# treangenlab/komb

Hardware: AMD Instinct MI355X
Metric: peeled edges/sec (k-truss) (higher is better)
Workload: dtype int32

## Files before the change

### komb_amd/csrc/ktruss.hip

```cpp
#include "peel_dev.h"
#include "truss_tail.h"
#include "local_dev.h"
#include "shard_dev.h"

#include <algorithm>
#include <cstdlib>
#include <cstring>

#include "truss_line.h"
#include "truss_tri.h"
#include "truss_wedge.h"
#include "truss_index.h"
#include "truss_gather.h"

namespace komb {

namespace {

struct TrussProblem {
    static constexpr bool kChain = false;
    static constexpr bool kSingleStep = false;
    uint32_t units;
    const uint2 *off2;
    const int2 *inc;
// ... 209 lines not shown
        }
        ctx->d_ceu = eu; ctx->d_cev = ev;
    }
    ctx->d_t_eu = ctx->d_ceu; ctx->d_t_ev = ctx->d_cev;
    return KOMB_OK;
}

int truss_support_canonical(komb_ctx *ctx)
{
    if (ctx->t_sup_ready) return KOMB_OK;
    if (!ctx->truss_done || !ctx->d_t_slice || !ctx->prep.valid || ctx->prep.ne != ctx->t_ne)
        KOMB_FAIL(ctx, KOMB_ERR_STATE, "komb_truss_fetch_support: no k-truss result to take the supports from");
    hipStream_t s = ctx->stream;
    const int64_t m = ctx->t_ne;
    KOMB_HIP(ctx, ctx->pool.get((void **)&ctx->d_t_sup, (size_t)m * sizeof(int32_t)));
#ifndef KOMB_TEST_SKIP_SLICE_ZERO
    if (ctx->t_k_lo) KOMB_HIP(ctx, hipMemsetAsync(ctx->d_t_sup, 0, (size_t)ctx->t_k_lo * sizeof(int32_t), s));
    if (ctx->t_k_hi < (uint32_t)m) KOMB_HIP(ctx, hipMemsetAsync(ctx->d_t_sup + ctx->t_k_hi, 0, ((size_t)m - ctx->t_k_hi) * sizeof(int32_t), s));
#endif
    k_scatter_len<<<grid_for(m), kBlock, 0, s>>>(ctx->d_t_slice, ctx->prep.e2k, m, ctx->t_k_lo, ctx->t_k_hi, ctx->d_t_sup);
    KOMB_HIP(ctx, hipStreamSynchronize(s));
    ctx->t_sup_ready = true;
    return KOMB_OK;
}

int truss_run(komb_ctx *ctx, const uint8_t *vmask_host, int rank, int world, komb_allreduce_fn fn, void *user)
{
    if (world < 1 || rank < 0 || rank >= world || (world > 1 && !fn))
        KOMB_FAIL(ctx, KOMB_ERR_ARG, "komb_truss_run_sharded: bad rank %d / world %d / callback", rank, world);
    if (ctx->nv < 0) KOMB_FAIL(ctx, KOMB_ERR_STATE, "komb_truss_run: no graph loaded");
    truss_free(ctx);
    hipStream_t s = ctx->stream;
    komb_stats &st = ctx->stats;
    st.triangles = 0; st.truss_levels = st.truss_subrounds = st.truss_launches = 0;
    st.max_trussness = 0; st.ms_support = st.ms_peel = st.ms_orient = st.ms_tri_count = st.ms_tri_fill = st.ms_gather = st.ms_allreduce = st.ms_compact = 0.0;
    st.truss_scans = 0; st.ms_prepare = 0.0; st.truss_prepared = 0; st.ms_prep_vertex = st.ms_prep_edges = st.ms_prep_rows = 0.0;
    auto empty_result = [&]() -> int {
        KOMB_HIP(ctx, ctx->pool.get((void **)&ctx->d_t_eu, 4)); KOMB_HIP(ctx, ctx->pool.get((void **)&ctx->d_t_ev, 4));
        KOMB_HIP(ctx, ctx->pool.get((void **)&ctx->d_t_truss, 4)); KOMB_HIP(ctx, ctx->pool.get((void **)&ctx->d_t_sup, 4));
        ctx->t_own_edges = true; ctx->t_ne = 0; ctx->truss_done = true; ctx->t_sup_ready = true;
        return KOMB_OK;
    };
    if (ctx->nv == 0 || ctx->ne == 0) return empty_result();
    Range r_all("komb_truss_run");
    DevBufs bufs(ctx);

    Range phase("truss: preparation");
    InducedCsr sub;
    TrussPrep sub_prep;
    struct SubGuard { komb_ctx *c; InducedCsr *g; TrussPrep *p; ~SubGuard() { prep_free(c, p); induced_free(c, g); } } sub_guard{ctx, &sub, &sub_prep};
    TrussPrep *tp = &ctx->prep;
    if (vmask_host) {
        ctx->timer.start(s);
        KOMB_TRY(induce_csr(ctx, vmask_host, &sub));
        st.ms_orient = ctx->timer.stop(s);
        if (sub.ns == 0) return empty_result();
        KOMB_TRY(prep_build(ctx, sub.rowptr, sub.col, sub.nv, sub.ns, &sub_prep));
        st.ms_prepare = sub_prep.ms; st.truss_prepared = 1;
        st.ms_prep_vertex = sub_prep.ms_part[0]; st.ms_prep_edges = sub_prep.ms_part[1]; st.ms_prep_rows = sub_prep.ms_part[2];
        tp = &sub_prep;
    } else if (!ctx->prep.valid) {
        KOMB_TRY(prep_ensure(ctx));
        st.ms_prepare = ctx->prep.ms; st.truss_prepared = 1;
        st.ms_prep_vertex = ctx->prep.ms_part[0]; st.ms_prep_edges = ctx->prep.ms_part[1]; st.ms_prep_rows = ctx->prep.ms_part[2];
    }
    const int64_t nv = tp->nv;
    const int64_t m = tp->ne;
    const uint32_t *d_orow = tp->orow;
    const int32_t *d_ocol = tp->ocol;
    const uint4 *d_line = tp->vline;
    const uint2 *d_wtasks = (const uint2 *)tp->wtasks;
    const int64_t n_wtasks = tp->n_wtasks;
    const int gw = grid_for(n_wtasks, kTriWaves);
    phase.next("truss: triangles + incidence index");

    const int ge = grid_for(m);
    const int tri_tv = (int)std::max<int64_t>(1, std::min<int64_t>(kTriV, nv / (256 * KOMB_TRI_EU * kTriWaves * 4)));
    const int64_t ntasks = (nv + tri_tv - 1) / tri_tv;
    const int gt = grid_for(ntasks, kTriWaves);
    uint32_t *d_own = nullptr, *d_other = nullptr, *d_cnt = nullptr, *d_off = nullptr;
    uint2 *d_off2 = nullptr;
    KOMB_HIP(ctx, bufs.alloc(&d_own, 2 * ((size_t)m + 1)));
    d_other = d_own + ((size_t)m + 1);
    KOMB_HIP(ctx, bufs.alloc(&d_cnt, (size_t)m + 1));
    KOMB_HIP(ctx, bufs.alloc(&d_off2, (size_t)m + 4));
    unsigned long long *d_mom = nullptr;
    KOMB_HIP(ctx, bufs.alloc(&d_mom, 12));
    KOMB_HIP(ctx, hipMemsetAsync(d_mom, 0, 12 * sizeof(unsigned long long), s));
    st.ms_allreduce = 0.0;

    const FinishMode fin = finish_mode(ctx, FIN_LOCAL);
    if (fin == FIN_LDS) KOMB_TRY(prep_sources(ctx, tp));
    const int32_t *d_osrc = tp->osrc;
    uint32_t tail_limit = 0;
    if (fin == FIN_LDS) {
        tail_limit = kTailEdges;
        if (const char *tl = ctx_opt(ctx, "TAIL")) tail_limit = (uint32_t)strtoul(tl, nullptr, 10);
        if (tail_limit > kTailMaxEdges) tail_limit = kTailMaxEdges;
    } else if (fin == FIN_LOCAL) tail_limit = local_limit(ctx, (uint64_t)m, 32);
    const bool whole_peel_finish = tail_limit && (uint64_t)m <= tail_limit;
    const bool shard_peel_on = (ctx->shard_peel && world > 1) || ctx_flag(ctx, "SHARD_ENGINE");
    enum { IDX_STREAM = 0, IDX_TWO_PASS = 2 };
    int layout = IDX_STREAM;
    if (const char *ix = ctx_opt(ctx, "INDEX")) {
        if (!strcmp(ix, "two_pass")) layout = IDX_TWO_PASS;
        else if (strcmp(ix, "stream")) KOMB_FAIL(ctx, KOMB_ERR_ARG, "option INDEX=%s: expected stream or two_pass", ix);
    }
    int2 *d_owndense = nullptr;
    unsigned long long *d_ownoff = nullptr, *d_dcur = nullptr;
    uint32_t *d_cnt_ref = nullptr;
    uint32_t *d_toff = nullptr;
    uint32_t *d_grp = nullptr;
    int32_t *d_light0 = nullptr;
    uint32_t *d_bintot = nullptr;
    uint32_t *d_reckey = nullptr;
    int2 *d_recval = nullptr;
    const BinGeom geom = bin_geom(m);
    const int64_t n_bins = (int64_t)geom.nb;
    const TriStream no_stream{nullptr, nullptr, nullptr, 0ull, 0u, 0u, 0};
#ifdef KOMB_DEBUG_SWITCHES
    const int ablate = getenv("KOMB_TRI_ABLATE") ? atoi(getenv("KOMB_TRI_ABLATE")) : 0;
#else
    const int ablate = 0;
#endif
    st.ms_sort = 0.0; st.tri_records = 0; st.ms_compact = 0.0; st.ms_tri_count = 0.0; st.ms_tri_fill = 0.0; st.stream_retries = 0;
    st.index_layout = layout;
    auto zero_counts = [&]() -> hipError_t { return hipMemsetAsync(d_own, 0, 2 * ((size_t)m + 1) * sizeof(uint32_t), s); };
    if (!(world == 1 && layout == IDX_STREAM)) KOMB_HIP(ctx, zero_counts());
    bool have_counts = false;
    if (world > 1) {
        const int64_t task_lo = n_wtasks * rank / world, task_hi = n_wtasks * (rank + 1) / world;
        ctx->timer.start(s);
        k_wedges<TRI_COUNT><<<gw, kBlock, 0, s>>>(d_orow, d_ocol, d_line, d_wtasks, task_lo, task_hi, d_own, d_other, nullptr, nullptr, 0ull, nullptr, no_stream, nullptr, ablate);
        st.ms_tri_count = ctx->timer.stop(s);
        k_sum_counts<<<ge, kBlock, 0, s>>>(d_own, d_other, nullptr, m + 1, d_cnt, d_mom + 5);
        ctx->timer.start(s);
        KOMB_HIP(ctx, hipStreamSynchronize(s));
        if (fn(user, d_cnt, (int64_t)m + 1) != 0)
            KOMB_FAIL(ctx, KOMB_ERR_DEVICE, "komb_truss_run_sharded: all-reduce callback failed");
        st.ms_allreduce = ctx->timer.stop(s);
        KOMB_HIP(ctx, hipMemsetAsync(d_mom + 5, 0, sizeof(unsigned long long), s));
        k_total_u32<<<ge, kBlock, 0, s>>>(d_cnt, m + 1, d_mom + 5);
        have_counts = true;
        if (layout != IDX_TWO_PASS) {
            KOMB_HIP(ctx, bufs.alloc(&d_cnt_ref, (size_t)m + 1));
            KOMB_HIP(ctx, hipMemcpyAsync(d_cnt_ref, d_cnt, ((size_t)m + 1) * sizeof(uint32_t), hipMemcpyDeviceToDevice, s));
            KOMB_HIP(ctx, zero_counts());
        }
    }

    if (layout == IDX_STREAM) {
        const unsigned long long bound = (unsigned long long)tp->own_bound;
        const int gws = std::min(gw, 256 * KOMB_WEDGE_EU);
        const unsigned long long slack = (unsigned long long)gws * kTriWaves * kRecChunk + kRecChunk;
        const unsigned long long own_slack = (unsigned long long)gws * kTriWaves * kOwnChunk + kOwnChunk;
        const unsigned long long t_bound = bound / 2;
        const unsigned long long own_full = bound + bound / 8 + own_slack, rec_full = 3 * t_bound + (3 * t_bound) / 14 + slack;
        unsigned long long own_cap = std::min(own_full, 4ull * (unsigned long long)m + own_slack);
        unsigned long long rec_cap = std::min(rec_full, 2ull * (unsigned long long)m + slack);
        bool fixed_caps = false;
        if (const char *oc = ctx_opt(ctx, "OWN_DENSE_CAP")) { own_cap = strtoull(oc, nullptr, 10) + 1; rec_cap = rec_full; fixed_caps = true; }
        if (ctx_flag(ctx, "NO_OWN_DENSE")) { own_cap = 1; rec_cap = rec_full; fixed_caps = true; }
        if (const char *rc = ctx_opt(ctx, "REC_CAP")) { rec_cap = strtoull(rc, nullptr, 10) + 1; fixed_caps = true; }
        if (ctx_flag(ctx, "FULL_CAPS")) { own_cap = own_full; rec_cap = rec_full; }
        if (!fixed_caps && ctx->cap_hint.nv == nv && ctx->cap_hint.m == m) {
            own_cap = std::min(own_full, std::max(own_cap, ctx->cap_hint.own_cap));
            rec_cap = std::min(rec_full, std::max(rec_cap, ctx->cap_hint.rec_cap));
        }
        const uint32_t sentinel = geom.sentinel_base();
        uint32_t *d_key = nullptr; int2 *d_val = nullptr;
        unsigned long long n_claimed = 0;
        bool ok = false;
        st.ms_tri_fill = 0.0;
        for (int attempt = 0; attempt < 2; ++attempt) {
            size_t free_b = 0, total_b = 0;
            (void)hipMemGetInfo(&free_b, &total_b);
            const unsigned long long budget = (unsigned long long)((free_b + ctx->pool.unused_bytes()) * 0.7);
            if (own_cap * sizeof(int2) > budget / 2) own_cap = budget / 2 / sizeof(int2);
            if (rec_cap * 12ull > budget / 2) rec_cap = budget / 2 / 12ull;
            if (rec_cap > 0xFFFFFFF0ull) rec_cap = 0xFFFFFFF0ull;
            ok = bufs.alloc(&d_key, (size_t)rec_cap) == hipSuccess && bufs.alloc(&d_val, (size_t)rec_cap) == hipSuccess &&
                 bufs.alloc(&d_owndense, (size_t)own_cap) == hipSuccess &&
                 (d_ownoff || bufs.alloc(&d_ownoff, (size_t)m + 1) == hipSuccess) && (d_dcur || bufs.alloc(&d_dcur, 4) == hipSuccess);
            uint2 *d_scratch = nullptr;
            if (ok && !ctx_flag(ctx, "NO_REC_SCRATCH") && bufs.alloc(&d_scratch, (size_t)gws * kTriWaves * kScratchRec) != hipSuccess) { (void)hipGetLastError(); d_scratch = nullptr; }
            if (!ok) { (void)hipGetLastError(); break; }
            KOMB_HIP(ctx, hipMemsetAsync(d_dcur, 0, 4 * sizeof(unsigned long long), s));
            const TriStream ts{d_key, d_val, d_dcur + 2, rec_cap, sentinel, geom.nb - 1u, kChunkBits};
            ctx->timer.start(s);
            k_wedges<TRI_SINGLE><<<gws, kBlock, 0, s>>>(d_orow, d_ocol, d_line, d_wtasks, 0, n_wtasks, d_own, d_other, d_owndense, d_dcur, own_cap, d_ownoff, ts, d_scratch, ablate);
            st.ms_tri_fill += ctx->timer.stop(s);
            unsigned long long dc[4] = {0, 0, 0, 0};
            KOMB_HIP(ctx, d2h(ctx, dc, d_dcur, sizeof(dc)));
            n_claimed = dc[2];
            bufs.release(d_scratch);
            if (ctx_flag(ctx, "TRI_DEBUG"))
                fprintf(stderr, "komb triangles: stream build (attempt %d): %llu record positions claimed of %llu, dense own-role region %llu entries claimed of %llu, %llu task ranges overflowed their record buffer\n",
                        attempt, dc[2], rec_cap, dc[0], own_cap, dc[1]);
            if (n_claimed <= rec_cap) {
                if (!fixed_caps) { ctx->cap_hint.nv = nv; ctx->cap_hint.m = m; ctx->cap_hint.own_cap = own_cap; ctx->cap_hint.rec_cap = rec_cap; }
                break;
            }
            ok = false;
            if (attempt == 1 || fixed_caps) break;
            bufs.release(d_key); bufs.release(d_val); bufs.release(d_owndense);
            d_key = nullptr; d_val = nullptr; d_owndense = nullptr;
            own_cap = std::min(own_full, std::max(own_cap, dc[0] + own_slack));
            rec_cap = std::min(rec_full, n_claimed + slack);
            st.stream_retries += 1;
        }
        uint32_t *d_skey = nullptr;
        if (ok) {
            uint32_t *d_key2 = nullptr; unsigned long long *d_val2 = nullptr;
            ok = bufs.alloc(&d_key2, (size_t)n_claimed + 1) == hipSuccess && bufs.alloc(&d_val2, (size_t)n_claimed + 1) == hipSuccess;
            if (ok) {
                ctx->timer.start(s);
                unsigned long long *sv = nullptr;
                if (geom.nb_bits > 0) KOMB_TRY(prim_sort_pairs_u32_u64(ctx, d_key, d_key2, (unsigned long long *)d_val, d_val2, (int64_t)n_claimed, kChunkBits, kChunkBits + geom.nb_bits, &d_skey, &sv));
                else { d_skey = d_key; sv = (unsigned long long *)d_val; }
                st.ms_sort = ctx->timer.stop(s);
                d_recval = (int2 *)sv;
                if (d_skey == d_key) { bufs.release(d_key2); bufs.release(d_val2); } else { bufs.release(d_key); bufs.release(d_val); }
                d_reckey = d_skey;
                KOMB_HIP(ctx, bufs.alloc(&d_toff, (size_t)n_bins + 2));
                KOMB_HIP(ctx, bufs.alloc(&d_bintot, (size_t)n_bins + 2));
                KOMB_HIP(ctx, bufs.alloc(&d_grp, (size_t)kInitOff + 4));
                if (!whole_peel_finish && !shard_peel_on && !ctx_flag(ctx, "NO_FIRST_QUEUE")) KOMB_HIP(ctx, bufs.alloc(&d_light0, (size_t)m));
                ctx->timer.start(s);
                peel_ctrl_pre(s, d_grp);
                KOMB_HIP(ctx, hipMemsetAsync(d_mom + 5, 0, sizeof(unsigned long long), s));
                k_bin_offsets<<<grid_for(n_bins + 1), kBlock, 0, s>>>(d_skey, (int64_t)n_claimed, geom, d_toff);
                k_bin_count<<<grid_for(n_bins, 1, 256 * 8), kBlock, 0, s>>>(d_skey, d_toff, geom, d_own, m, d_cnt, d_bintot, d_mom + 5, (int32_t *)(d_grp + kInitOff + 1));
                st.ms_compact = ctx->timer.stop(s);
                st.tri_records = (int64_t)n_claimed;
            } else (void)hipGetLastError();
        }
        if (!ok) {
            bufs.release(d_key); bufs.release(d_val); bufs.release(d_owndense); bufs.release(d_ownoff); bufs.release(d_dcur);
            bufs.release(d_grp); bufs.release(d_light0); d_grp = nullptr; d_light0 = nullptr;
            d_owndense = nullptr; d_ownoff = nullptr; d_dcur = nullptr;
            KOMB_HIP(ctx, zero_counts());
            KOMB_HIP(ctx, hipMemsetAsync(d_mom + 5, 0, sizeof(unsigned long long), s));
            st.ms_tri_fill = 0.0;
            layout = IDX_TWO_PASS;
        }
    }
    if (layout != IDX_TWO_PASS && d_cnt_ref) {
        k_count_mismatch<<<ge, kBlock, 0, s>>>(d_cnt, d_cnt_ref, m + 1, d_mom + 8);
    }
    if (layout == IDX_TWO_PASS) {
        if (d_cnt_ref) {
            KOMB_HIP(ctx, hipMemcpyAsync(d_cnt, d_cnt_ref, ((size_t)m + 1) * sizeof(uint32_t), hipMemcpyDeviceToDevice, s));
            KOMB_HIP(ctx, hipMemsetAsync(d_mom + 5, 0, sizeof(unsigned long long), s));
            k_total_u32<<<ge, kBlock, 0, s>>>(d_cnt, m + 1, d_mom + 5);
        } else if (!have_counts) {
            ctx->timer.start(s);
            k_triangles<TRI_COUNT><<<gt, kBlock, 0, s>>>(d_orow, d_ocol, nv, 0, ntasks, d_own, d_other, nullptr, nullptr, ablate, tri_tv);
            st.ms_tri_count = ctx->timer.stop(s);
            k_sum_counts<<<ge, kBlock, 0, s>>>(d_own, d_other, nullptr, m + 1, d_cnt, d_mom + 5);
        }
    }
    st.index_layout = layout;
    {
        unsigned long long mom[9];
        KOMB_HIP(ctx, d2h(ctx, mom, d_mom, sizeof(mom)));
        st.triangles = (int64_t)(mom[5] / 3);
        bufs.release(d_mom);
        if (mom[8] != 0)
            KOMB_FAIL(ctx, KOMB_ERR_DEVICE, "komb_truss_run_sharded: %llu edges whose all-reduced support differs from the support of the index build", mom[8]);
        if (mom[5] > 0xFFFFFFF0ull)
            KOMB_FAIL(ctx, KOMB_ERR_LIMIT, "graph has %llu triangles; the incidence index is limited to 2^32-16 entries (3 per triangle)",
                      mom[5] / 3);
    }
    bufs.release(d_cnt_ref);
    uint32_t total = 0;
    const uint32_t sum_supports = (uint32_t)st.triangles * 3u;
    int2 *d_inc = nullptr;
    int32_t *d_sup = nullptr, *d_stamp = nullptr, *d_truss = nullptr;
    uint8_t *d_st8 = nullptr;
    bool peel_inited = false;
    if (layout == IDX_STREAM) {
        KOMB_TRY(prim_exclusive_sum_u32(ctx, d_bintot, d_bintot, n_bins + 1));
        total = sum_supports;
        KOMB_HIP(ctx, bufs.alloc(&d_inc, (size_t)total));
        KOMB_HIP(ctx, bufs.alloc(&d_sup, (size_t)m));
        KOMB_HIP(ctx, bufs.alloc(&d_stamp, (size_t)m));
        KOMB_HIP(ctx, bufs.alloc(&d_st8, (size_t)m + 16));
        KOMB_HIP(ctx, bufs.alloc(&d_truss, (size_t)m));
        ctx->timer.start(s);
        k_bin_finish<<<grid_for(n_bins, 1, 256 * kFinPerCu), kFinBlock, 0, s>>>(d_reckey, d_recval, d_toff, geom, d_own, d_cnt, d_bintot, d_owndense, d_ownoff, d_inc, m,
                                                                      d_off2, d_sup, d_stamp, d_st8, d_grp + kInitOff, d_light0);
        st.ms_compact += ctx->timer.stop(s);
        peel_inited = true;
        bufs.release(d_toff); bufs.release(d_bintot); bufs.release((void *)d_recval); bufs.release(d_reckey);
        bufs.release(d_owndense); bufs.release(d_ownoff); bufs.release(d_dcur);
    } else {
        KOMB_HIP(ctx, bufs.alloc(&d_off, (size_t)m + 1));
        KOMB_TRY(prim_exclusive_sum_u32(ctx, d_cnt, d_off, m + 1));
        KOMB_HIP(ctx, d2h(ctx, &total, d_off + m, sizeof(uint32_t)));
        KOMB_HIP(ctx, bufs.alloc(&d_inc, (size_t)total));
        ctx->timer.start(s);
        KOMB_HIP(ctx, zero_counts());
        k_back_cursors<<<ge, kBlock, 0, s>>>(d_off, m, d_other);
        k_triangles<TRI_SINGLE><<<gt, kBlock, 0, s>>>(d_orow, d_ocol, nv, 0, ntasks, d_own, d_other, d_off, d_inc, ablate, tri_tv);
        st.ms_tri_fill = ctx->timer.stop(s);
    }
    st.ms_support = st.ms_tri_count + st.ms_tri_fill + st.ms_sort + st.ms_compact;
    bufs.release(d_cnt); bufs.release(d_own);

    phase.next("truss: peel");
    PeelCtrl *d_ctrl = nullptr;
    PeelQueues Q{nullptr, {nullptr, nullptr}, {nullptr, nullptr}, {nullptr, nullptr}, 0};
    const size_t heavy_cap = (size_t)total / 32 + 64;
    if (!peel_inited) {
        KOMB_HIP(ctx, bufs.alloc(&d_sup, (size_t)m));
        KOMB_HIP(ctx, bufs.alloc(&d_stamp, (size_t)m));
        KOMB_HIP(ctx, bufs.alloc(&d_st8, (size_t)m + 16));
        KOMB_HIP(ctx, bufs.alloc(&d_truss, (size_t)m));
        KOMB_HIP(ctx, bufs.alloc(&d_grp, (size_t)kInitOff + 4));
    }
    for (int i = 0; i < 2; ++i) {
        if (i == 0 && d_light0) Q.light[0] = d_light0;
        else KOMB_HIP(ctx, bufs.alloc(&Q.light[i], (size_t)m));
        KOMB_HIP(ctx, bufs.alloc(&Q.heavy[i], heavy_cap));
        KOMB_HIP(ctx, bufs.alloc(&Q.live[i], (size_t)m / 2 + 64));
    }
    KOMB_HIP(ctx, bufs.alloc(&d_ctrl, 1));
    KOMB_HIP(ctx, bufs.alloc(&Q.code, (size_t)m));
    KOMB_HIP(ctx, bufs.alloc(&Q.rlevel, (size_t)m + 2));
    KOMB_HIP(ctx, hipMemsetAsync(Q.rlevel, 0, 2 * sizeof(int32_t), s));
    int32_t retire_every = kRetireEvery;
    if (const char *e = ctx_opt(ctx, "RETIRE_EVERY")) retire_every = std::max(1, std::min((int)kRetireEvery, atoi(e)));
#ifdef KOMB_DEBUG_SWITCHES
    TrussProblem P{(uint32_t)m, d_off2, d_inc, d_sup, d_stamp, d_st8, retire_every, getenv("KOMB_PEEL_ABLATE") ? atoi(getenv("KOMB_PEEL_ABLATE")) : 0};
#else
    TrussProblem P{(uint32_t)m, d_off2, d_inc, d_sup, d_stamp, d_st8, retire_every};
#endif
    TailBufs T{};
    if (fin == FIN_LDS && tail_limit) {
        KOMB_HIP(ctx, bufs.alloc(&T.vmap, (size_t)nv));
        KOMB_HIP(ctx, bufs.alloc(&T.cnt, 64));
        KOMB_HIP(ctx, bufs.alloc(&T.vlist, (size_t)kTailMaxV));
        KOMB_HIP(ctx, bufs.alloc(&T.rows, (size_t)kTailMaxV * kTailRowWords));
        KOMB_HIP(ctx, bufs.alloc(&T.pair, (size_t)tail_limit));
        KOMB_HIP(ctx, bufs.alloc(&T.sup, (size_t)tail_limit));
        KOMB_HIP(ctx, bufs.alloc(&T.gid, (size_t)tail_limit));
        KOMB_HIP(ctx, bufs.alloc(&T.gid_by_rank, (size_t)tail_limit));
        KOMB_HIP(ctx, bufs.alloc(&T.pair_by_rank, (size_t)tail_limit));
        KOMB_HIP(ctx, bufs.alloc(&T.truss_by_rank, (size_t)tail_limit));
        KOMB_HIP(ctx, bufs.alloc(&T.spill[0], (size_t)tail_limit));
        KOMB_HIP(ctx, bufs.alloc(&T.spill[1], (size_t)tail_limit));
        T.max_edges = tail_limit;
    }
    auto run_tail = [&](const int32_t *list, uint32_t n_in) -> int {
        KOMB_HIP(ctx, hipMemsetAsync(T.vmap, 0, (size_t)nv * sizeof(int32_t), s));
        KOMB_HIP(ctx, hipMemsetAsync(T.cnt, 0, 64 * sizeof(uint32_t), s));
        KOMB_HIP(ctx, hipMemsetAsync(T.rows, 0, (size_t)kTailMaxV * kTailRowWords * sizeof(unsigned long long), s));
        const int g = grid_for(n_in, kBlock, 256);
        const bool dbg = ctx_flag(ctx, "TAIL_DEBUG");
        hipEvent_t ev[3] = {nullptr, nullptr, nullptr};
        for (auto &e : ev) (void)hipEventCreate(&e);
        (void)hipEventRecord(ev[0], s);
        k_tail_mark<<<g, kBlock, 0, s>>>(list, n_in, d_sup, d_stamp, d_osrc, d_ocol, T);
        k_tail_number<<<1, kTailMaxV, 0, s>>>(T);
        k_tail_rows<<<g, kBlock, 0, s>>>(list, n_in, d_sup, d_stamp, d_osrc, d_ocol, T);
        (void)hipEventRecord(ev[1], s);
        k_truss_tail<<<1, 1024, 0, s>>>(d_ctrl, T, d_truss);
        (void)hipEventRecord(ev[2], s);
        KOMB_HIP(ctx, d2h(ctx, &ctx->h_ctrl[0], d_ctrl, sizeof(PeelCtrl)));
        ++st.truss_tail_runs;
        float m0 = 0, m1 = 0, m2 = 0;
        (void)hipEventElapsedTime(&m0, ctx->timer.a, ev[0]); (void)hipEventElapsedTime(&m1, ev[0], ev[1]); (void)hipEventElapsedTime(&m2, ev[1], ev[2]);
        for (auto &e : ev) (void)hipEventDestroy(e);
        st.ms_tail += (double)m1 + (double)m2;
        if (dbg) {
            uint32_t h[16];
            KOMB_HIP(ctx, d2h(ctx, h, T.cnt, sizeof(h)));
            fprintf(stderr, "komb tail: %u vertices, %u edges, %s; general engine before it %.1f us, setup %.1f us, tail kernel %.1f us\n",
                    h[0], h[1], ctx->h_ctrl[0].done == 1 ? "done" : "refused", m0 * 1000.f, m1 * 1000.f, m2 * 1000.f);
#ifdef KOMB_TAIL_TIMERS
            fprintf(stderr, "komb tail: us in kernel: load %.1f ranks %.1f supports %.1f scan %.1f mark %.1f triangles %.1f retire %.1f results %.1f\n",
                    h[14] / 100.0, h[15] / 100.0, h[8] / 100.0, h[9] / 100.0, h[10] / 100.0, h[11] / 100.0, h[12] / 100.0, h[13] / 100.0);
#endif
        }
        return KOMB_OK;
    };
    const int gp = peel_grid(m);
    auto run_local = [&]() -> int {
        const PeelCtrl hc = ctx->h_ctrl[0];
// ... 145 lines not shown
```

### komb_amd/csrc/truss_index.h

```cpp
#pragma once

#include "peel_dev.h"

namespace komb {

namespace {

constexpr int kBinBits = 11;
constexpr uint32_t kBinEdges = 1u << kBinBits;
#ifndef KOMB_CHUNK_BITS
#define KOMB_CHUNK_BITS 6
#endif
constexpr int kChunkBits = KOMB_CHUNK_BITS;
constexpr uint32_t kChunkMask = (1u << kChunkBits) - 1u;
struct BinGeom {
    int nb_bits;
    uint32_t nb;
    __host__ __device__ uint32_t bin_of(uint32_t e) const { return (e >> kChunkBits) & (nb - 1u); }
    __host__ __device__ uint32_t local_of(uint32_t e) const { return ((e >> (kChunkBits + nb_bits)) << kChunkBits) | (e & kChunkMask); }
    __host__ __device__ uint64_t edge_of(uint32_t b, uint32_t i) const
    {
        return ((((uint64_t)(i >> kChunkBits) << nb_bits) | b) << kChunkBits) | (i & kChunkMask);
    }
    __host__ __device__ uint32_t sentinel_base() const { return (uint32_t)(((uint64_t)kBinEdges >> kChunkBits) << (kChunkBits + nb_bits)); }
};
inline BinGeom bin_geom(int64_t m)
{
    BinGeom g{0, 1u};
    while (((int64_t)g.nb << kBinBits) < m) { ++g.nb_bits; g.nb <<= 1; }
    return g;
}

__global__ __launch_bounds__(kBlock) void k_bin_offsets(const uint32_t *__restrict__ key, int64_t n, BinGeom g, uint32_t *__restrict__ boff)
{
    for (int64_t b = (int64_t)blockIdx.x * kBlock + threadIdx.x; b <= (int64_t)g.nb; b += (int64_t)gridDim.x * kBlock) {
        int64_t lo = 0, hi = n;
        while (lo < hi) {
            const int64_t mid = lo + ((hi - lo) >> 1);
            if ((int64_t)g.bin_of(key[mid]) < b) lo = mid + 1; else hi = mid;
        }
        boff[b] = (uint32_t)lo;
    }
}

__global__ __launch_bounds__(kBlock) void k_count_mismatch(const uint32_t *__restrict__ a, const uint32_t *__restrict__ b, int64_t n,
                                                           unsigned long long *__restrict__ bad)
{
    unsigned long long t = 0;
    for (int64_t e = (int64_t)blockIdx.x * kBlock + threadIdx.x; e < n; e += (int64_t)gridDim.x * kBlock) t += a[e] != b[e] ? 1ull : 0ull;
    block_add_u64(t, bad);
}

__global__ __launch_bounds__(kBlock) void k_bin_count(const uint32_t *__restrict__ key, const uint32_t *__restrict__ boff, BinGeom g,
                                                      const uint32_t *__restrict__ own, int64_t m, uint32_t *__restrict__ sum,
                                                      uint32_t *__restrict__ bin_total, unsigned long long *__restrict__ total,
                                                      int32_t *__restrict__ min_pos)
{
    __shared__ uint32_t sh_cnt[kBinEdges];
    __shared__ uint32_t sh_part[kBlock / kWave];
    unsigned long long t = 0;
    int32_t lmin = 0x7FFFFFFF;
    for (uint32_t b = blockIdx.x; b < g.nb; b += gridDim.x) {
        for (uint32_t i = threadIdx.x; i < kBinEdges; i += kBlock) sh_cnt[i] = 0u;
        __syncthreads();
        const uint32_t r0 = boff[b], r1 = boff[b + 1];
        for (uint32_t r = r0 + threadIdx.x; r < r1; r += kBlock) {
            const uint32_t k = key[r];
            if ((int64_t)k < m) atomicAdd(&sh_cnt[g.local_of(k)], 1u);
        }
        __syncthreads();
        uint32_t tb = 0;
        for (uint32_t i = threadIdx.x; i < kBinEdges; i += kBlock) {
            const uint64_t e = g.edge_of(b, i);
            if (e >= (uint64_t)m) continue;
            const uint32_t c = own[e] + sh_cnt[i];
            sum[e] = c;
            tb += c;
            if (c) lmin = min(lmin, (int32_t)c);
        }
        tb = wave_sum(tb);
        if (lane_id() == 0) sh_part[threadIdx.x >> 6] = tb;
        __syncthreads();
        if (threadIdx.x == 0) {
            uint32_t all = 0;
            for (int i = 0; i < kBlock / kWave; ++i) all += sh_part[i];
            bin_total[b] = all;
            t += all;
        }
        __syncthreads();
    }
    if (blockIdx.x == 0 && threadIdx.x == 0) { sum[m] = 0u; bin_total[g.nb] = 0u; }
    if (threadIdx.x == 0 && t) atomicAdd(total, t);
    lmin = wave_min(lmin);
    if (lane_id() == 0 && lmin != 0x7FFFFFFF) atomicMin(min_pos, lmin);
}

constexpr int kFinBlock = 512;
#ifndef KOMB_FIN_PER_CU
#define KOMB_FIN_PER_CU 2
#endif
#ifndef KOMB_WIN_CAP
#define KOMB_WIN_CAP 7168
#endif
constexpr int kFinPerCu = KOMB_FIN_PER_CU;
constexpr uint32_t kWinCap = KOMB_WIN_CAP;
constexpr int kFinE = (int)(kBinEdges / kFinBlock);
constexpr int kFinU = 4;
static_assert((kWinCap * 8 + 2 * kBinEdges * 4 + 512) * kFinPerCu <= 160 * 1024, "the finishing workgroups of a CU: windows and tables are sized for gfx950's 160 KB of LDS");
static_assert(kWinCap * 8 >= (2 * kBinEdges + 4) * 4 + kBinEdges * 8, "the window buffer doubles as the table of the in-place copy");
static_assert(kFinE == 4 && kFinE <= (1 << kChunkBits), "a thread's edges are 4 consecutive ones of a chunk: their supports and own-role counts are one 16-byte vector each");
__global__ __launch_bounds__(kFinBlock, (kFinBlock / 64) * kFinPerCu / 4) void k_bin_finish(const uint32_t *__restrict__ key, const int2 *__restrict__ val,
                                                         const uint32_t *__restrict__ boff, BinGeom g,
                                                         const uint32_t *__restrict__ own, const uint32_t *__restrict__ cnt,
                                                         const uint32_t *__restrict__ bin_base,
                                                         const int2 *__restrict__ own_dense, const unsigned long long *__restrict__ ownoff,
                                                         int2 *__restrict__ dense, int64_t m,
                                                         uint2 *__restrict__ off2, int32_t *__restrict__ sup, int32_t *__restrict__ stamp, uint8_t *__restrict__ st8,
                                                         uint32_t *__restrict__ init, int32_t *__restrict__ light0)
{
    __shared__ uint32_t sh_off[kBinEdges + 4];
    __shared__ uint32_t sh_cur[kBinEdges];
    __shared__ uint32_t sh_wsum[kFinBlock / kWave];
    __shared__ int2 sh_win[kWinCap];
    __shared__ uint32_t sh_hsum[kFinBlock / kWave];
    __shared__ uint32_t sh_qbase;
    const int lane = lane_id(), w = (int)(threadIdx.x >> 6);
    uint32_t zeros = 0;
    const int32_t L1 = (int32_t)init[1];
    const bool queue_first = light0 != nullptr && L1 <= kLight;
    for (uint32_t b = blockIdx.x; b < g.nb; b += gridDim.x) {
        const uint64_t r0 = boff[b], r1 = boff[b + 1];
        const uint32_t base = bin_base[b];
        const uint32_t i0 = threadIdx.x * (uint32_t)kFinE;
        const uint64_t e0 = g.edge_of(b, i0);
        const uint32_t nin = e0 >= (uint64_t)m ? 0u : (uint32_t)min((uint64_t)kFinE, (uint64_t)m - e0);
        uint32_t c[kFinE], ow[kFinE];
        unsigned long long oo[kFinE];
        if (nin == (uint32_t)kFinE) {
            const uint4 v = *reinterpret_cast<const uint4 *>(cnt + e0);
            const uint4 q = *reinterpret_cast<const uint4 *>(own + e0);
            c[0] = v.x; c[1] = v.y; c[2] = v.z; c[3] = v.w;
            ow[0] = q.x; ow[1] = q.y; ow[2] = q.z; ow[3] = q.w;
        } else {
#pragma unroll
            for (int u = 0; u < kFinE; ++u) { const bool in = (uint32_t)u < nin; c[u] = in ? cnt[e0 + u] : 0u; ow[u] = in ? own[e0 + u] : 0u; }
        }
#pragma unroll
        for (int u = 0; u < kFinE; ++u) oo[u] = ow[u] ? ownoff[e0 + u] : 0ull;
        const uint32_t mine = c[0] + c[1] + c[2] + c[3];
        const uint32_t incl = wave_incl_scan(mine);
        uint32_t hits = 0;
#pragma unroll
        for (int u = 0; u < kFinE; ++u) hits += (queue_first && (int32_t)c[u] == L1) ? 1u : 0u;
        const uint32_t hincl = wave_incl_scan(hits);
        if (lane == kWave - 1) { sh_wsum[w] = incl; sh_hsum[w] = hincl; }
        __syncthreads();
        uint32_t before = 0, hbefore = 0, hall = 0;
#pragma unroll
        for (int i = 0; i < kFinBlock / kWave; ++i) { before += i < w ? sh_wsum[i] : 0u; hbefore += i < w ? sh_hsum[i] : 0u; hall += sh_hsum[i]; }
        if (threadIdx.x == 0 && hall) sh_qbase = atomicAdd(&init[2], hall);
        uint32_t o[kFinE + 1];
        o[0] = before + incl - mine;
#pragma unroll
        for (int u = 0; u < kFinE; ++u) o[u + 1] = o[u] + c[u];
#pragma unroll
        for (int u = 0; u < kFinE; ++u) { sh_off[i0 + u] = o[u]; sh_cur[i0 + u] = o[u]; }
        if (threadIdx.x == kFinBlock - 1) sh_off[kBinEdges] = o[kFinE];
        if (nin == (uint32_t)kFinE) {
            reinterpret_cast<uint4 *>(off2 + e0)[0] = make_uint4(base + o[0], c[0], base + o[1], c[1]);
            reinterpret_cast<uint4 *>(off2 + e0)[1] = make_uint4(base + o[2], c[2], base + o[3], c[3]);
            int4 sv, mv;
            int32_t *svp = &sv.x, *mvp = &mv.x;
#pragma unroll
            for (int u = 0; u < kFinE; ++u) {
                const bool first = queue_first && (int32_t)c[u] == L1;
                svp[u] = (int32_t)c[u];
                mvp[u] = first ? 1 : (c[u] ? alive_marker(c[u]) : 0);
                if (!c[u]) ++zeros;
            }
            *reinterpret_cast<int4 *>(sup + e0) = sv;
            *reinterpret_cast<int4 *>(stamp + e0) = mv;
            *reinterpret_cast<uchar4 *>(st8 + e0) = make_uchar4(state_of_stamp(mv.x), state_of_stamp(mv.y), state_of_stamp(mv.z), state_of_stamp(mv.w));
        } else {
#pragma unroll
            for (int u = 0; u < kFinE; ++u) if ((uint32_t)u < nin) {
                const uint64_t e = e0 + u;
                const bool first = queue_first && (int32_t)c[u] == L1;
                off2[e] = make_uint2(base + o[u], c[u]);
                sup[e] = (int32_t)c[u];
                stamp[e] = first ? 1 : (c[u] ? alive_marker(c[u]) : 0);
                st8[e] = state_of_stamp(stamp[e]);
                if (!c[u]) ++zeros;
            }
        }
        __syncthreads();
        if (hall) {
            uint32_t q = sh_qbase + hbefore + hincl - hits;
#pragma unroll
            for (int u = 0; u < kFinE; ++u) if (queue_first && (int32_t)c[u] == L1 && (uint32_t)u < nin) light0[q++] = (int32_t)(e0 + u);
        }
        const uint32_t W = sh_off[kBinEdges];
        const bool inwin = W <= kWinCap;
        for (uint64_t r = r0 + threadIdx.x; r < r1; r += (uint64_t)kFinBlock * kFinU) {
            uint32_t k[kFinU];
            int2 v[kFinU];
#pragma unroll
            for (int u = 0; u < kFinU; ++u) {
                const uint64_t rr = r + (uint64_t)u * kFinBlock;
                if (rr < r1) { k[u] = key[rr]; v[u] = val[rr]; }
            }
#pragma unroll
            for (int u = 0; u < kFinU; ++u) {
                const uint64_t rr = r + (uint64_t)u * kFinBlock;
                if (rr < r1 && (int64_t)k[u] < m) {
                    const uint32_t p = atomicAdd(&sh_cur[g.local_of(k[u])], 1u);
                    if (inwin) sh_win[p] = v[u]; else dense[base + p] = v[u];
                }
            }
        }
        if (inwin) {
            uint32_t most = 0;
#pragma unroll
            for (int u = 0; u < kFinE; ++u) most = max(most, ow[u]);
            for (uint32_t kk = 0; kk < most; ++kk) {
                int2 t[kFinE];
#pragma unroll
                for (int u = 0; u < kFinE; ++u) if (kk < ow[u]) t[u] = own_dense[oo[u] + kk];
#pragma unroll
                for (int u = 0; u < kFinE; ++u) if (kk < ow[u]) sh_win[o[u + 1] - ow[u] + kk] = t[u];
            }
        } else {
            uint32_t *tab_pre = reinterpret_cast<uint32_t *>(sh_win), *tab_dst = tab_pre + kBinEdges + 4;
            unsigned long long *tab_src = reinterpret_cast<unsigned long long *>(tab_dst + kBinEdges);
            const uint32_t mine_ow = ow[0] + ow[1] + ow[2] + ow[3];
            const uint32_t incl_ow = wave_incl_scan(mine_ow);
            __syncthreads();
            if (lane == kWave - 1) sh_wsum[w] = incl_ow;
            __syncthreads();
            uint32_t before_ow = 0, total_ow = 0;
#pragma unroll
            for (int i = 0; i < kFinBlock / kWave; ++i) { before_ow += i < w ? sh_wsum[i] : 0u; total_ow += sh_wsum[i]; }
            uint32_t run = before_ow + incl_ow - mine_ow;
#pragma unroll
            for (int u = 0; u < kFinE; ++u) {
                tab_pre[i0 + u] = run; tab_dst[i0 + u] = o[u + 1] - ow[u]; tab_src[i0 + u] = oo[u];
                run += ow[u];
            }
            if (threadIdx.x == kFinBlock - 1) tab_pre[kBinEdges] = run;
            __syncthreads();
            for (uint32_t x = threadIdx.x; x < total_ow; x += kFinBlock) {
                uint32_t lo = 0;
#pragma unroll
                for (uint32_t st = kBinEdges / 2; st > 0; st >>= 1) lo += (tab_pre[lo + st] <= x) ? st : 0u;
                const uint32_t kk = x - tab_pre[lo];
                dense[base + tab_dst[lo] + kk] = own_dense[tab_src[lo] + kk];
            }
        }
        __syncthreads();
        if (inwin) for (uint32_t j = threadIdx.x; j < W; j += kFinBlock) dense[base + j] = sh_win[j];
        __syncthreads();
    }
    block_add_min(zeros, 0x7FFFFFFF, &init[0], (int32_t *)&init[1]);
}

__global__ __launch_bounds__(kBlock) void k_peel_init(int64_t m, const uint32_t *__restrict__ off, uint2 *__restrict__ off2,
                                                      int32_t *__restrict__ sup, int32_t *__restrict__ stamp, uint8_t *__restrict__ st8,
                                                      uint32_t *__restrict__ init)
{
    uint32_t zeros = 0;
    int32_t lmin = 0x7FFFFFFF;
    for (int64_t e = (int64_t)blockIdx.x * kBlock + threadIdx.x; e < m; e += (int64_t)gridDim.x * kBlock) {
        const uint32_t b0 = off[e];
        const int32_t s0 = (int32_t)(off[e + 1] - b0);
        off2[e] = make_uint2(b0, (uint32_t)s0);
        sup[e] = s0;
        if (s0 == 0) { stamp[e] = 0; st8[e] = (uint8_t)ST_GONE; ++zeros; }
        else { const int32_t a = alive_marker((uint32_t)s0); stamp[e] = a; st8[e] = state_of_stamp(a); lmin = min(lmin, s0); }
    }
    block_add_min(zeros, lmin, &init[0], (int32_t *)&init[1]);
}

}

}
```

Baseline: 4.039 billion.

## Fuse per-edge support counting into bin finish and drop the count pass

Removes the separate k_bin_count kernel and its global per-edge count array. Support counts are now accumulated in shared memory inside k_bin_finish, and the kernel also reduces the support total and minimum. A new wave-per-bin k_bin_bounds kernel replaces k_bin_offsets and computes each bin's window size from record count plus own-role sum. This lets the index be sized from an upper bound before exact triangle counts are known, saving a full pass over the keys and an m-sized buffer. The cost is a possibly over-allocated index, a device-to-host read before finish, and the first-frontier threshold fixed to 1 instead of read from init.

Measured after the change: 4.068 billion, median of 5. About the same (+0.7%).

```diff
diff --git a/komb_amd/csrc/ktruss.hip b/komb_amd/csrc/ktruss.hip
--- a/komb_amd/csrc/ktruss.hip
+++ b/komb_amd/csrc/ktruss.hip
@@ -315,7 +315,6 @@
     uint2 *d_off2 = nullptr;
     KOMB_HIP(ctx, bufs.alloc(&d_own, 2 * ((size_t)m + 1)));
     d_other = d_own + ((size_t)m + 1);
-    KOMB_HIP(ctx, bufs.alloc(&d_cnt, (size_t)m + 1));
     KOMB_HIP(ctx, bufs.alloc(&d_off2, (size_t)m + 4));
     unsigned long long *d_mom = nullptr;
     KOMB_HIP(ctx, bufs.alloc(&d_mom, 12));
@@ -345,7 +344,10 @@
     uint32_t *d_toff = nullptr;
     uint32_t *d_grp = nullptr;
     int32_t *d_light0 = nullptr;
-    uint32_t *d_bintot = nullptr;
+    uint32_t *d_binwin = nullptr;
+    unsigned long long stream_extent = 0;
+    EventSet evs;
+    hipEvent_t ev_idx[5] = {nullptr, nullptr, nullptr, nullptr, nullptr};
     uint32_t *d_reckey = nullptr;
     int2 *d_recval = nullptr;
     const BinGeom geom = bin_geom(m);
@@ -361,6 +363,7 @@
     auto zero_counts = [&]() -> hipError_t { return hipMemsetAsync(d_own, 0, 2 * ((size_t)m + 1) * sizeof(uint32_t), s); };
     if (!(world == 1 && layout == IDX_STREAM)) KOMB_HIP(ctx, zero_counts());
     bool have_counts = false;
+    if (world > 1 || layout == IDX_TWO_PASS) KOMB_HIP(ctx, bufs.alloc(&d_cnt, (size_t)m + 1));
     if (world > 1) {
         const int64_t task_lo = n_wtasks * rank / world, task_hi = n_wtasks * (rank + 1) / world;
         ctx->timer.start(s);
@@ -447,24 +450,26 @@
             uint32_t *d_key2 = nullptr; unsigned long long *d_val2 = nullptr;
             ok = bufs.alloc(&d_key2, (size_t)n_claimed + 1) == hipSuccess && bufs.alloc(&d_val2, (size_t)n_claimed + 1) == hipSuccess;
             if (ok) {
-                ctx->timer.start(s);
+                for (auto &e : ev_idx) KOMB_HIP(ctx, evs.make(&e));
+                (void)hipEventRecord(ev_idx[0], s);
                 unsigned long long *sv = nullptr;
                 if (geom.nb_bits > 0) KOMB_TRY(prim_sort_pairs_u32_u64(ctx, d_key, d_key2, (unsigned long long *)d_val, d_val2, (int64_t)n_claimed, kChunkBits, kChunkBits + geom.nb_bits, &d_skey, &sv));
                 else { d_skey = d_key; sv = (unsigned long long *)d_val; }
-                st.ms_sort = ctx->timer.stop(s);
+                (void)hipEventRecord(ev_idx[1], s);
                 d_recval = (int2 *)sv;
                 if (d_skey == d_key) { bufs.release(d_key2); bufs.release(d_val2); } else { bufs.release(d_key); bufs.release(d_val); }
                 d_reckey = d_skey;
                 KOMB_HIP(ctx, bufs.alloc(&d_toff, (size_t)n_bins + 2));
-                KOMB_HIP(ctx, bufs.alloc(&d_bintot, (size_t)n_bins + 2));
+                KOMB_HIP(ctx, bufs.alloc(&d_binwin, (size_t)n_bins + 2));
                 KOMB_HIP(ctx, bufs.alloc(&d_grp, (size_t)kInitOff + 4));
                 if (!whole_peel_finish && !shard_peel_on && !ctx_flag(ctx, "NO_FIRST_QUEUE")) KOMB_HIP(ctx, bufs.alloc(&d_light0, (size_t)m));
-                ctx->timer.start(s);
                 peel_ctrl_pre(s, d_grp);
-                KOMB_HIP(ctx, hipMemsetAsync(d_mom + 5, 0, sizeof(unsigned long long), s));
-                k_bin_offsets<<<grid_for(n_bins + 1), kBlock, 0, s>>>(d_skey, (int64_t)n_claimed, geom, d_toff);
-                k_bin_count<<<grid_for(n_bins, 1, 256 * 8), kBlock, 0, s>>>(d_skey, d_toff, geom, d_own, m, d_cnt, d_bintot, d_mom + 5, (int32_t *)(d_grp + kInitOff + 1));
-                st.ms_compact = ctx->timer.stop(s);
+                KOMB_HIP(ctx, hipMemsetAsync(d_mom + 5, 0, 2 * sizeof(unsigned long long), s));
+                k_bin_bounds<<<grid_for(n_bins, kBlock / kWave), kBlock, 0, s>>>(d_skey, (int64_t)n_claimed, geom, d_own, m, d_toff, d_binwin, d_mom + 6);
+                (void)hipEventRecord(ev_idx[2], s);
+                unsigned long long own_sum = 0;
+                KOMB_HIP(ctx, d2h(ctx, &own_sum, d_mom + 6, sizeof(own_sum)));
+                stream_extent = n_claimed + own_sum;
                 st.tri_records = (int64_t)n_claimed;
             } else (void)hipGetLastError();
         }
@@ -472,14 +477,12 @@
             bufs.release(d_key); bufs.release(d_val); bufs.release(d_owndense); bufs.release(d_ownoff); bufs.release(d_dcur);
             bufs.release(d_grp); bufs.release(d_light0); d_grp = nullptr; d_light0 = nullptr;
             d_owndense = nullptr; d_ownoff = nullptr; d_dcur = nullptr;
+            if (!d_cnt) KOMB_HIP(ctx, bufs.alloc(&d_cnt, (size_t)m + 1));
             KOMB_HIP(ctx, zero_counts());
             KOMB_HIP(ctx, hipMemsetAsync(d_mom + 5, 0, sizeof(unsigned long long), s));
             st.ms_tri_fill = 0.0;
             layout = IDX_TWO_PASS;
         }
-    }
-    if (layout != IDX_TWO_PASS && d_cnt_ref) {
-        k_count_mismatch<<<ge, kBlock, 0, s>>>(d_cnt, d_cnt_ref, m + 1, d_mom + 8);
     }
     if (layout == IDX_TWO_PASS) {
         if (d_cnt_ref) {
@@ -494,7 +497,7 @@
         }
     }
     st.index_layout = layout;
-    {
+    auto read_moments = [&]() -> int {
         unsigned long long mom[9];
         KOMB_HIP(ctx, d2h(ctx, mom, d_mom, sizeof(mom)));
         st.triangles = (int64_t)(mom[5] / 3);
@@ -504,30 +507,41 @@
         if (mom[5] > 0xFFFFFFF0ull)
             KOMB_FAIL(ctx, KOMB_ERR_LIMIT, "graph has %llu triangles; the incidence index is limited to 2^32-16 entries (3 per triangle)",
                       mom[5] / 3);
-    }
-    bufs.release(d_cnt_ref);
+        return KOMB_OK;
+    };
     uint32_t total = 0;
-    const uint32_t sum_supports = (uint32_t)st.triangles * 3u;
     int2 *d_inc = nullptr;
     int32_t *d_sup = nullptr, *d_stamp = nullptr, *d_truss = nullptr;
     uint8_t *d_st8 = nullptr;
     bool peel_inited = false;
     if (layout == IDX_STREAM) {
-        KOMB_TRY(prim_exclusive_sum_u32(ctx, d_bintot, d_bintot, n_bins + 1));
-        total = sum_supports;
+        if (stream_extent > 0xFFFFFFF0ull)
+            KOMB_FAIL(ctx, KOMB_ERR_LIMIT, "graph needs up to %llu entries of the incidence index (3 per triangle, the exact number of triangles is not known at this point); the index is limited to 2^32-16 entries",
+                      stream_extent);
+        KOMB_TRY(prim_exclusive_sum_u32(ctx, d_binwin, d_binwin, n_bins));
+        total = (uint32_t)stream_extent;
         KOMB_HIP(ctx, bufs.alloc(&d_inc, (size_t)total));
         KOMB_HIP(ctx, bufs.alloc(&d_sup, (size_t)m));
         KOMB_HIP(ctx, bufs.alloc(&d_stamp, (size_t)m));
         KOMB_HIP(ctx, bufs.alloc(&d_st8, (size_t)m + 16));
         KOMB_HIP(ctx, bufs.alloc(&d_truss, (size_t)m));
-        ctx->timer.start(s);
-        k_bin_finish<<<grid_for(n_bins, 1, 256 * kFinPerCu), kFinBlock, 0, s>>>(d_reckey, d_recval, d_toff, geom, d_own, d_cnt, d_bintot, d_owndense, d_ownoff, d_inc, m,
-                                                                      d_off2, d_sup, d_stamp, d_st8, d_grp + kInitOff, d_light0);
-        st.ms_compact += ctx->timer.stop(s);
+        (void)hipEventRecord(ev_idx[3], s);
+        k_bin_finish<<<grid_for(n_bins, 1, 256 * kFinPerCu), kFinBlock, 0, s>>>(d_reckey, d_recval, d_toff, geom, d_own, d_binwin, d_owndense, d_ownoff, d_inc, m,
+                                                                      d_off2, d_sup, d_stamp, d_st8, d_grp + kInitOff, d_light0, d_mom + 5);
+        (void)hipEventRecord(ev_idx[4], s);
+        if (d_cnt_ref) k_count_mismatch<<<ge, kBlock, 0, s>>>((const uint32_t *)d_sup, d_cnt_ref, m, d_mom + 8);
+        KOMB_TRY(read_moments());
+        float ms_idx[3] = {0.f, 0.f, 0.f};
+        (void)hipEventElapsedTime(&ms_idx[0], ev_idx[0], ev_idx[1]);
+        (void)hipEventElapsedTime(&ms_idx[1], ev_idx[1], ev_idx[2]);
+        (void)hipEventElapsedTime(&ms_idx[2], ev_idx[3], ev_idx[4]);
+        st.ms_sort = (double)ms_idx[0];
+        st.ms_compact = (double)ms_idx[1] + (double)ms_idx[2];
         peel_inited = true;
-        bufs.release(d_toff); bufs.release(d_bintot); bufs.release((void *)d_recval); bufs.release(d_reckey);
+        bufs.release(d_toff); bufs.release(d_binwin); bufs.release((void *)d_recval); bufs.release(d_reckey);
         bufs.release(d_owndense); bufs.release(d_ownoff); bufs.release(d_dcur);
     } else {
+        KOMB_TRY(read_moments());
         KOMB_HIP(ctx, bufs.alloc(&d_off, (size_t)m + 1));
         KOMB_TRY(prim_exclusive_sum_u32(ctx, d_cnt, d_off, m + 1));
         KOMB_HIP(ctx, d2h(ctx, &total, d_off + m, sizeof(uint32_t)));
@@ -538,6 +552,7 @@
         k_triangles<TRI_SINGLE><<<gt, kBlock, 0, s>>>(d_orow, d_ocol, nv, 0, ntasks, d_own, d_other, d_off, d_inc, ablate, tri_tv);
         st.ms_tri_fill = ctx->timer.stop(s);
     }
+    bufs.release(d_cnt_ref);
     st.ms_support = st.ms_tri_count + st.ms_tri_fill + st.ms_sort + st.ms_compact;
     bufs.release(d_cnt); bufs.release(d_own);
 
diff --git a/komb_amd/csrc/truss_index.h b/komb_amd/csrc/truss_index.h
--- a/komb_amd/csrc/truss_index.h
+++ b/komb_amd/csrc/truss_index.h
@@ -31,16 +31,34 @@
     return g;
 }
 
-__global__ __launch_bounds__(kBlock) void k_bin_offsets(const uint32_t *__restrict__ key, int64_t n, BinGeom g, uint32_t *__restrict__ boff)
-{
-    for (int64_t b = (int64_t)blockIdx.x * kBlock + threadIdx.x; b <= (int64_t)g.nb; b += (int64_t)gridDim.x * kBlock) {
-        int64_t lo = 0, hi = n;
+__global__ __launch_bounds__(kBlock) void k_bin_bounds(const uint32_t *__restrict__ key, int64_t n, BinGeom g, const uint32_t *__restrict__ own, int64_t m,
+                                                       uint32_t *__restrict__ boff, uint32_t *__restrict__ bin_ext, unsigned long long *__restrict__ own_total)
+{
+    constexpr int kWaves = kBlock / kWave;
+    const int lane = lane_id();
+    unsigned long long t = 0;
+    for (int64_t b = (int64_t)blockIdx.x * kWaves + (threadIdx.x >> 6); b < (int64_t)g.nb; b += (int64_t)gridDim.x * kWaves) {
+        int64_t lo = 0, hi = lane < 2 ? n : 0;
         while (lo < hi) {
             const int64_t mid = lo + ((hi - lo) >> 1);
-            if ((int64_t)g.bin_of(key[mid]) < b) lo = mid + 1; else hi = mid;
-        }
-        boff[b] = (uint32_t)lo;
-    }
+            if ((int64_t)g.bin_of(key[mid]) < b + lane) lo = mid + 1; else hi = mid;
+        }
+        const uint32_t first = (uint32_t)__shfl((int)lo, 0), next = (uint32_t)__shfl((int)lo, 1);
+        uint32_t o = 0;
+#pragma unroll 8
+        for (uint32_t c = 0; c < kBinEdges / kWave; ++c) {
+            const uint64_t e = g.edge_of((uint32_t)b, c * kWave + (uint32_t)lane);
+            if (e < (uint64_t)m) o += own[e];
+        }
+        o = wave_sum(o);
+        if (lane == 0) {
+            boff[b] = first;
+            if (b + 1 == (int64_t)g.nb) boff[b + 1] = next;
+            bin_ext[b] = (next - first) + o;
+            t += o;
+        }
+    }
+    block_add_u64(t, own_total);
 }
 
 __global__ __launch_bounds__(kBlock) void k_count_mismatch(const uint32_t *__restrict__ a, const uint32_t *__restrict__ b, int64_t n,
@@ -49,50 +67,6 @@
     unsigned long long t = 0;
     for (int64_t e = (int64_t)blockIdx.x * kBlock + threadIdx.x; e < n; e += (int64_t)gridDim.x * kBlock) t += a[e] != b[e] ? 1ull : 0ull;
     block_add_u64(t, bad);
-}
-
-__global__ __launch_bounds__(kBlock) void k_bin_count(const uint32_t *__restrict__ key, const uint32_t *__restrict__ boff, BinGeom g,
-                                                      const uint32_t *__restrict__ own, int64_t m, uint32_t *__restrict__ sum,
-                                                      uint32_t *__restrict__ bin_total, unsigned long long *__restrict__ total,
-                                                      int32_t *__restrict__ min_pos)
-{
-    __shared__ uint32_t sh_cnt[kBinEdges];
-    __shared__ uint32_t sh_part[kBlock / kWave];
-    unsigned long long t = 0;
-    int32_t lmin = 0x7FFFFFFF;
-    for (uint32_t b = blockIdx.x; b < g.nb; b += gridDim.x) {
-        for (uint32_t i = threadIdx.x; i < kBinEdges; i += kBlock) sh_cnt[i] = 0u;
-        __syncthreads();
-        const uint32_t r0 = boff[b], r1 = boff[b + 1];
-        for (uint32_t r = r0 + threadIdx.x; r < r1; r += kBlock) {
-            const uint32_t k = key[r];
-            if ((int64_t)k < m) atomicAdd(&sh_cnt[g.local_of(k)], 1u);
-        }
-        __syncthreads();
-        uint32_t tb = 0;
-        for (uint32_t i = threadIdx.x; i < kBinEdges; i += kBlock) {
-            const uint64_t e = g.edge_of(b, i);
-            if (e >= (uint64_t)m) continue;
-            const uint32_t c = own[e] + sh_cnt[i];
-            sum[e] = c;
-            tb += c;
-            if (c) lmin = min(lmin, (int32_t)c);
-        }
-        tb = wave_sum(tb);
-        if (lane_id() == 0) sh_part[threadIdx.x >> 6] = tb;
-        __syncthreads();
-        if (threadIdx.x == 0) {
-            uint32_t all = 0;
-            for (int i = 0; i < kBlock / kWave; ++i) all += sh_part[i];
-            bin_total[b] = all;
-            t += all;
-        }
-        __syncthreads();
-    }
-    if (blockIdx.x == 0 && threadIdx.x == 0) { sum[m] = 0u; bin_total[g.nb] = 0u; }
-    if (threadIdx.x == 0 && t) atomicAdd(total, t);
-    lmin = wave_min(lmin);
-    if (lane_id() == 0 && lmin != 0x7FFFFFFF) atomicMin(min_pos, lmin);
 }
 
 constexpr int kFinBlock = 512;
@@ -111,12 +85,11 @@
 static_assert(kFinE == 4 && kFinE <= (1 << kChunkBits), "a thread's edges are 4 consecutive ones of a chunk: their supports and own-role counts are one 16-byte vector each");
 __global__ __launch_bounds__(kFinBlock, (kFinBlock / 64) * kFinPerCu / 4) void k_bin_finish(const uint32_t *__restrict__ key, const int2 *__restrict__ val,
                                                          const uint32_t *__restrict__ boff, BinGeom g,
-                                                         const uint32_t *__restrict__ own, const uint32_t *__restrict__ cnt,
-                                                         const uint32_t *__restrict__ bin_base,
+                                                         const uint32_t *__restrict__ own, const uint32_t *__restrict__ bin_base,
                                                          const int2 *__restrict__ own_dense, const unsigned long long *__restrict__ ownoff,
                                                          int2 *__restrict__ dense, int64_t m,
                                                          uint2 *__restrict__ off2, int32_t *__restrict__ sup, int32_t *__restrict__ stamp, uint8_t *__restrict__ st8,
-                                                         uint32_t *__restrict__ init, int32_t *__restrict__ light0)
+                                                         uint32_t *__restrict__ init, int32_t *__restrict__ light0, unsigned long long *__restrict__ sup_total)
 {
     __shared__ uint32_t sh_off[kBinEdges + 4];
     __shared__ uint32_t sh_cur[kBinEdges];
@@ -126,8 +99,11 @@
     __shared__ uint32_t sh_qbase;
     const int lane = lane_id(), w = (int)(threadIdx.x >> 6);
     uint32_t zeros = 0;
-    const int32_t L1 = (int32_t)init[1];
-    const bool queue_first = light0 != nullptr && L1 <= kLight;
+    int32_t lmin = 0x7FFFFFFF;
+    uint32_t tsum = 0;
+    constexpr int32_t L1 = 1;
+    static_assert(L1 <= kLight, "the first frontier is queued as light units");
+    const bool queue_first = light0 != nullptr;
     for (uint32_t b = blockIdx.x; b < g.nb; b += gridDim.x) {
         const uint64_t r0 = boff[b], r1 = boff[b + 1];
         const uint32_t base = bin_base[b];
@@ -137,17 +113,35 @@
         uint32_t c[kFinE], ow[kFinE];
         unsigned long long oo[kFinE];
         if (nin == (uint32_t)kFinE) {
-            const uint4 v = *reinterpret_cast<const uint4 *>(cnt + e0);
             const uint4 q = *reinterpret_cast<const uint4 *>(own + e0);
-            c[0] = v.x; c[1] = v.y; c[2] = v.z; c[3] = v.w;
             ow[0] = q.x; ow[1] = q.y; ow[2] = q.z; ow[3] = q.w;
         } else {
 #pragma unroll
-            for (int u = 0; u < kFinE; ++u) { const bool in = (uint32_t)u < nin; c[u] = in ? cnt[e0 + u] : 0u; ow[u] = in ? own[e0 + u] : 0u; }
+            for (int u = 0; u < kFinE; ++u) ow[u] = (uint32_t)u < nin ? own[e0 + u] : 0u;
+        }
+#pragma unroll
+        for (int u = 0; u < kFinE; ++u) sh_cur[i0 + u] = 0u;
+        __syncthreads();
+        for (uint64_t r = r0 + threadIdx.x; r < r1; r += (uint64_t)kFinBlock * kFinU) {
+            uint32_t k[kFinU];
+#pragma unroll
+            for (int u = 0; u < kFinU; ++u) {
+                const uint64_t rr = r + (uint64_t)u * kFinBlock;
+                k[u] = rr < r1 ? key[rr] : 0xFFFFFFFFu;
+            }
+#pragma unroll
+            for (int u = 0; u < kFinU; ++u) if ((int64_t)k[u] < m) atomicAdd(&sh_cur[g.local_of(k[u])], 1u);
         }
 #pragma unroll
         for (int u = 0; u < kFinE; ++u) oo[u] = ow[u] ? ownoff[e0 + u] : 0ull;
+        __syncthreads();
+#pragma unroll
+        for (int u = 0; u < kFinE; ++u) {
+            c[u] = ow[u] + sh_cur[i0 + u];
+            if (c[u]) lmin = min(lmin, (int32_t)c[u]);
+        }
         const uint32_t mine = c[0] + c[1] + c[2] + c[3];
+        tsum += mine;
         const uint32_t incl = wave_incl_scan(mine);
         uint32_t hits = 0;
 #pragma unroll
@@ -260,7 +254,8 @@
         if (inwin) for (uint32_t j = threadIdx.x; j < W; j += kFinBlock) dense[base + j] = sh_win[j];
         __syncthreads();
     }
-    block_add_min(zeros, 0x7FFFFFFF, &init[0], (int32_t *)&init[1]);
+    block_add_min(zeros, lmin, &init[0], (int32_t *)&init[1]);
+    block_add_u64((unsigned long long)tsum, sup_total);
 }
 
 __global__ __launch_bounds__(kBlock) void k_peel_init(int64_t m, const uint32_t *__restrict__ off, uint2 *__restrict__ off2,
```
